# mahyarnajibi/SNIPER

Measured on AMD Instinct MI355X. Metric: train chips/sec (512x512, R101), higher is better.
Workload: dtype f16; 1 GPU; ResNet-101 Faster-RCNN SNIPER 3-scale, batch 20 x 512x512 fp16 per GPU (BASELINE configs[1]); step = GPU anchor labelling + fwd + bwd + grad all-reduce + SGD on HBM-resident chips (epoch chip generation / box assignment and image decode+resize are outside the step); f16 MFMA operands, f32 accumulation / losses / master weights; chips_per_gpu=20, global_batch=20, parallelism=dp1

## Files before the change

sniper_amd/csrc/common.h:

```cpp
#pragma once
#include <hip/hip_runtime.h>
#include <stdint.h>
#include <stdio.h>
#include <stdlib.h>

#include "../../include/sniper_hip.h"

#define SN_EXPORT extern "C" __attribute__((visibility("default")))

void sn_set_error(const char *fmt, ...);

#define SN_REQUIRE(cond, ...)      \
  do {                             \
    if (!(cond)) {                 \
      sn_set_error(__VA_ARGS__);   \
      return SN_ERR_ARG;           \
    }                              \
  } while (0)

#define SN_CHECK_LAUNCH()                                                      \
  do {                                                                         \
    hipError_t e__ = hipGetLastError();                                        \
    if (e__ != hipSuccess) {                                                   \
      sn_set_error("%s:%d HIP launch failed: %s", __FILE__, __LINE__, hipGetErrorString(e__)); \
      return SN_ERR_HIP;                                                       \
    }                                                                          \
  } while (0)

#define SN_HIP(call)                                                           \
  do {                                                                         \
    hipError_t e__ = (call);                                                   \
    if (e__ != hipSuccess) {                                                   \
      sn_set_error("%s:%d %s: %s", __FILE__, __LINE__, #call, hipGetErrorString(e__)); \
      return SN_ERR_HIP;                                                       \
    }                                                                          \
  } while (0)

hipError_t sn_once_per_device_max_lds(const void *kernel, int bytes);
enum SnDebugOption { SN_OPT_PROPOSAL_FULL_SORT = 0, SN_OPT_NMS_FULL_MASK = 1, SN_OPT_CONV_NO_PERSIST = 2, SN_OPT_SOFTMAX_STRIDED = 3, SN_OPT_COUNT };
int sn_debug_get(SnDebugOption which);

static inline hipStream_t sn_stream(sn_stream_t s) { return (hipStream_t)s; }
static inline int sn_div_up(int a, int b) { return (a + b - 1) / b; }
static inline size_t sn_align(size_t x, size_t a = 256) { return (x + a - 1) / a * a; }

static inline int sn_env_int(const char *name, int dflt) {
  const char *v = getenv(name);
  return v && *v ? atoi(v) : dflt;
}
static inline int sn_conv_out(int in, int k, int stride, int pad, int dil) { return (in + 2 * pad - dil * (k - 1) - 1) / stride + 1; }
static inline int sn_blocks(long total, int cap) {
  const long b = (total + 255) / 256;
  return (int)(b < 1 ? 1 : (b > cap ? cap : b));
}

constexpr int kWave = 64;

typedef _Float16 half_t;
typedef _Float16 half8 __attribute__((ext_vector_type(8)));
typedef _Float16 half4 __attribute__((ext_vector_type(4)));
typedef float floatx4 __attribute__((ext_vector_type(4)));

__device__ __forceinline__ unsigned sn_float_key(float f) {
  const unsigned u = __float_as_uint(f);
  return (u & 0x80000000u) ? ~u : (u | 0x80000000u);
}

int sn_partial_sum(const float *part, int nblk, long n, float *dst, hipStream_t s);

struct SnDiv { unsigned mul, sh, d; };
static inline SnDiv sn_div_make(unsigned d) {
  SnDiv f;
  unsigned s = 0;
  while ((1ull << s) < d) ++s;
  f.mul = (unsigned)((((unsigned long long)1 << 32) * (((unsigned long long)1 << s) - d)) / d + 1);
  f.sh = s;
  f.d = d;
  return f;
}
__device__ __forceinline__ unsigned sn_div(unsigned n, const SnDiv f) { return (__umulhi(n, f.mul) + n) >> f.sh; }
__device__ __forceinline__ unsigned sn_divmod(unsigned n, const SnDiv f, unsigned &rem) {
  const unsigned q = sn_div(n, f);
  rem = n - q * f.d;
  return q;
}
```

sniper_amd/csrc/common.hip:

```cpp
#include "common.h"

#include <stdarg.h>
#include <stdlib.h>
#include <string.h>

#include <atomic>
#include <mutex>
#include <string>
#include <utility>
#include <vector>

static thread_local char g_err[512] = "";

void sn_set_error(const char *fmt, ...) {
  va_list ap;
  va_start(ap, fmt);
  vsnprintf(g_err, sizeof(g_err), fmt, ap);
  va_end(ap);
}

SN_EXPORT const char *sn_last_error(void) { return g_err; }
SN_EXPORT int sn_version(void) { return 100; }

hipError_t sn_once_per_device_max_lds(const void *kernel, int bytes) {
  static std::mutex mu;
  static std::vector<std::pair<const void *, int>> done;
  int dev = 0;
  hipError_t e = hipGetDevice(&dev);
  if (e != hipSuccess) return e;
  std::lock_guard<std::mutex> lock(mu);
  for (const auto &d : done)
    if (d.first == kernel && d.second == dev) return hipSuccess;
  e = hipFuncSetAttribute(kernel, hipFuncAttributeMaxDynamicSharedMemorySize, bytes);
  if (e == hipSuccess) done.emplace_back(kernel, dev);
  return e;
}

static std::atomic<int> g_debug[SN_OPT_COUNT];
static const char *const kDebugNames[SN_OPT_COUNT] = {"proposal_full_sort", "nms_full_mask", "conv_no_persist", "softmax_strided"};
static const char *const kDebugEnv[SN_OPT_COUNT] = {"SNIPER_FULL_SORT", "SNIPER_NMS_FULL", "SNIPER_CONV_NO_PERSIST", "SNIPER_SOFTMAX_STRIDED"};
namespace {
struct DebugInit {
  DebugInit() {
    for (int i = 0; i < SN_OPT_COUNT; ++i) g_debug[i].store(getenv(kDebugEnv[i]) != nullptr ? 1 : 0, std::memory_order_relaxed);
  }
} g_debug_init;
}

int sn_debug_get(SnDebugOption which) { return g_debug[which].load(std::memory_order_relaxed); }

__global__ __launch_bounds__(256) void partial_sum_kernel(const float *__restrict__ part, int nblk, long n, float *__restrict__ dst) {
  const long e = (long)blockIdx.x * 256 + threadIdx.x;
  if (e >= n) return;
  float s = 0.f;
  int k = 0;
  for (; k + 8 <= nblk; k += 8) {
    float v[8];
#pragma unroll
    for (int u = 0; u < 8; ++u) v[u] = part[(size_t)(k + u) * n + e];
#pragma unroll
    for (int u = 0; u < 8; ++u) s += v[u];
  }
  for (; k < nblk; ++k) s += part[(size_t)k * n + e];
  dst[e] += s;
}

int sn_partial_sum(const float *part, int nblk, long n, float *dst, hipStream_t s) {
  hipLaunchKernelGGL(partial_sum_kernel, dim3((unsigned)((n + 255) / 256)), dim3(256), 0, s, part, nblk, n, dst);
  SN_CHECK_LAUNCH();
  return SN_OK;
}

SN_EXPORT int sn_debug_option(const char *name, int value) {
  SN_REQUIRE(name, "sn_debug_option: null name");
  for (int i = 0; i < SN_OPT_COUNT; ++i)
    if (strcmp(name, kDebugNames[i]) == 0) {
      g_debug[i].store(value, std::memory_order_relaxed);
      return SN_OK;
    }
  SN_REQUIRE(false, "sn_debug_option: unknown option '%s'", name);
}
```

sniper_amd/csrc/roi_deform.hip:

```cpp
#include "common.h"
#include "deform_sample.h"
#include <type_traits>

#include <stdlib.h>


struct RoiGeom {
  int b;
  float wstart, hstart, sub_w, sub_h, roi_w, roi_h;
};

__device__ __forceinline__ RoiGeom roi_geom(const float *__restrict__ rois, const float *__restrict__ trans, int r, int ph,
                                            int pw, int P, int S, float scale, float trans_std) {
#pragma clang fp contract(off)
  const float *q = rois + (size_t)r * 5;
  RoiGeom g;
  g.b = (int)q[0];
  const float sw = roundf(q[1]) * scale - 0.5f, sh = roundf(q[2]) * scale - 0.5f;
  const float ew = (roundf(q[3]) + 1.f) * scale - 0.5f, eh = (roundf(q[4]) + 1.f) * scale - 0.5f;
  g.roi_w = fmaxf(ew - sw, 0.1f);
  g.roi_h = fmaxf(eh - sh, 0.1f);
  const float bin_w = g.roi_w / (float)P, bin_h = g.roi_h / (float)P;
  g.sub_w = bin_w / (float)S;
  g.sub_h = bin_h / (float)S;
// ... 792 lines not shown
    const float wy = tent_sum(ay, y);
    if (wy == 0.f) continue;
    for (int x = ax.lo; x <= ax.hi; ++x) {
      const float wgt = wy * tent_sum(ax, x);
      if (wgt == 0.f) continue;
      sum += wgt * (float)img[((size_t)y * W + x) * C];
    }
  }
  return sum;
}

template <bool WAVE_PER_BIN>
__global__ __launch_bounds__(256) void psroi_ps_fwd_kernel(const half_t *__restrict__ data, const float *__restrict__ rois,
                                                           const float *__restrict__ trans, half_t *__restrict__ out, int R, int H,
                                                           int W, int C, int P, int S, int G, int D, float scale, float trans_std, int gm) {
  if constexpr (WAVE_PER_BIN) {
    const long total = (long)R * P * P;
    const long wv = ((long)blockIdx.x * blockDim.x + threadIdx.x) >> 6;
    if (wv >= total) return;
    const int lane = threadIdx.x & 63;
    const int pw = (int)(wv % P), ph = (int)((wv / P) % P), r = (int)(wv / ((long)P * P));
    const RoiGeom g = roi_geom(rois, trans, r, ph, pw, P, S, scale, trans_std);
    const AxisSamples ax = axis_samples(g.wstart, g.sub_w, S, W), ay = axis_samples(g.hstart, g.sub_h, S, H);
    const int count = ax.n * ay.n;
    const float inv = count ? 1.f / (float)count : 0.f;
    const int gh = ps_group(ph, G, P), gw = ps_group(pw, G, P);
    const half_t *img = data + (size_t)g.b * H * W * C;
    for (int d = lane; d < D; d += 64) {
      const float sum = count ? ps_bin_value(ax, ay, img + ps_channel(d, gh, gw, G, D, gm), W, C) : 0.f;
      out[(size_t)wv * D + d] = (half_t)(sum * inv);
    }
  } else {
    const long total = (long)R * P * P * D;
    for (long i = (long)blockIdx.x * blockDim.x + threadIdx.x; i < total; i += (long)gridDim.x * blockDim.x) {
      const int d = (int)(i % D);
      long t = i / D;
      const int pw = (int)(t % P); t /= P;
      const int ph = (int)(t % P);
      const int r = (int)(t / P);
      const RoiGeom g = roi_geom(rois, trans, r, ph, pw, P, S, scale, trans_std);
      const AxisSamples ax = axis_samples(g.wstart, g.sub_w, S, W), ay = axis_samples(g.hstart, g.sub_h, S, H);
      const int count = ax.n * ay.n;
      const int c = ps_channel(d, ps_group(ph, G, P), ps_group(pw, G, P), G, D, gm);
      const float sum = count ? ps_bin_value(ax, ay, data + (size_t)g.b * H * W * C + c, W, C) : 0.f;
      out[i] = (half_t)(count ? sum / (float)count : 0.f);
    }
  }
}

template <bool GM>
__global__ __launch_bounds__(256) void psroi_ps_bwd_data_kernel(const half_t *__restrict__ dout, const float *__restrict__ rois,
                                                                const float *__restrict__ trans, const int4 *__restrict__ win,
                                                                void *__restrict__ d_data, int out_f32, int R, int H, int W, int C,
                                                                int P, int S, int G, int D, float scale, float trans_std) {
  __shared__ __attribute__((aligned(16))) float ent[256 * kEntStride];
  __shared__ int roi_list[256];
  __shared__ int bins[256];
  __shared__ int wave_cnt[4], ent_cnt[4], nb_s;
  const int PP = P * P;
  const int tid = threadIdx.x, lane = tid & 63, wave = tid >> 6;
  const unsigned long long lt = (1ull << lane) - 1ull;
  int x0, y0;
  tile_origin(W, x0, y0);
  const int b = blockIdx.y;
  int c, d, mygrp, g_lo, g_hi;
  bool active_c;
  if constexpr (GM) {
    c = blockIdx.z * 256 + tid;
    active_c = c < C;
    mygrp = active_c ? c / D : -1;
    d = active_c ? c - mygrp * D : 0;
    g_lo = (blockIdx.z * 256) / D;
    g_hi = min(G * G - 1, (blockIdx.z * 256 + 255) / D);
  } else {
    const int chunks = (D + 255) >> 8;
    mygrp = g_lo = g_hi = blockIdx.z / chunks;
    d = (blockIdx.z % chunks) * 256 + tid;
    active_c = d < D;
    c = (d * G + mygrp / G) * G + mygrp % G;
  }
  if (tid == 0) {
    int n = 0;
    for (int bin = 0; bin < PP; ++bin) {
      const int grp = ps_group(bin / P, G, P) * G + ps_group(bin % P, G, P);
      if (grp >= g_lo && grp <= g_hi) bins[n++] = bin;
    }
    nb_s = n;
  }
  __syncthreads();
  const int nb = nb_s;
  float acc[16];
#pragma unroll
  for (int k = 0; k < 16; ++k) acc[k] = 0.f;
  if (nb > 0) {
    for (int base = 0; base < R; base += 256) {
      const int total = tile_scan_rois(win, base, R, b, x0, y0, roi_list, wave_cnt);
      const int nitems = total * nb;
      for (int it0 = 0; it0 < nitems; it0 += 256) {
        const int item = it0 + tid;
        bool act = false;
        float Wx[4] = {0.f, 0.f, 0.f, 0.f}, Wy[4] = {0.f, 0.f, 0.f, 0.f};
        float inv = 0.f;
        int idx = 0, grp = 0;
        if (item < nitems) {
          const int r = roi_list[item / nb], bin = bins[item % nb];
          const int ph = bin / P, pw = bin - ph * P;
          if constexpr (GM) grp = ps_group(ph, G, P) * G + ps_group(pw, G, P);
          act = bin_tile_weights(roi_geom(rois, trans, r, ph, pw, P, S, scale, trans_std), S, H, W, x0, y0, Wx, Wy, inv);
          idx = r * PP + bin;
        }
        const unsigned long long am = __ballot(act);
        if (lane == 0) ent_cnt[wave] = __popcll(am);
        __syncthreads();
        int eoff, n_e;
        wave_prefix4(ent_cnt, wave, eoff, n_e);
        if (act) {
          float *e = ent + (size_t)(eoff + __popcll(am & lt)) * kEntStride;
          e[0] = __int_as_float(idx);
          if constexpr (GM) e[1] = __int_as_float(grp);
          *reinterpret_cast<float4 *>(e + 4) = make_float4(Wx[0] * inv, Wx[1] * inv, Wx[2] * inv, Wx[3] * inv);
          *reinterpret_cast<float4 *>(e + 8) = make_float4(Wy[0], Wy[1], Wy[2], Wy[3]);
        }
        __syncthreads();
        if constexpr (GM) {
          for (int e = 0; e < n_e; ++e) {
            const float *q = ent + e * kEntStride;
            if (__float_as_int(q[1]) != mygrp) continue;
            tile_fma(q, (float)dout[(size_t)__float_as_int(q[0]) * D + d], acc);
          }
        } else {
          tile_accumulate<half_t>(ent, n_e, dout, (size_t)D, d, active_c, acc);
        }
        __syncthreads();
      }
    }
  }
  if (active_c) tile_store(acc, d_data, out_f32, b, y0, x0, H, W, C, c);
}

__global__ __launch_bounds__(256) void psroi_ps_bwd_trans_kernel(const half_t *__restrict__ dout, const half_t *__restrict__ data,
                                                                 const float *__restrict__ rois, const float *__restrict__ trans,
                                                                 float *__restrict__ d_trans, int R, int H, int W, int C, int P,
                                                                 int S, int G, int D, float scale, float trans_std, int gm) {
  const long total = (long)R * P * P;
  const long wv = ((long)blockIdx.x * blockDim.x + threadIdx.x) >> 6;
  if (wv >= total) return;
  const int lane = threadIdx.x & 63;
  const int pw = (int)(wv % P), ph = (int)((wv / P) % P), r = (int)(wv / ((long)P * P));
  const RoiGeom g = roi_geom(rois, trans, r, ph, pw, P, S, scale, trans_std);
  const int gh = ps_group(ph, G, P), gw = ps_group(pw, G, P);
  const half_t *img = data + (size_t)g.b * H * W * C;
  const AxisSamples ax = axis_samples(g.wstart, g.sub_w, S, W), ay = axis_samples(g.hstart, g.sub_h, S, H);
  const int count = ax.n * ay.n;
  const int nx = count ? ax.hi - ax.lo + 1 : 0, ny = count ? ay.hi - ay.lo + 1 : 0;
  float gtx = 0.f, gty = 0.f;
  if (count && nx <= kWinMax && ny <= kWinMax) {
    const int q = lane & 7;
    const bool is_y = (lane >> 3) & 1;
    const float wl = is_y ? (q < ny ? tent_sum(ay, ay.lo + q) : 0.f) : (q < nx ? tent_sum(ax, ax.lo + q) : 0.f);
    const float dl = is_y ? (q < ny ? tent_dsum(ay, ay.lo + q) : 0.f) : (q < nx ? tent_dsum(ax, ax.lo + q) : 0.f);
    for (int d = lane; d < D + 63 - ((D - 1) & 63); d += 64) {
      const bool on = d < D;
      const int c = ps_channel(on ? d : 0, gh, gw, G, D, gm);
      const float dv = on ? (float)dout[(size_t)wv * D + d] : 0.f;
      float sx = 0.f, sy = 0.f;
      for (int qy = 0; qy < ny; ++qy) {
        const float wy = __builtin_bit_cast(float, __builtin_amdgcn_readlane(__builtin_bit_cast(int, wl), 8 + qy));
        const float dwy = __builtin_bit_cast(float, __builtin_amdgcn_readlane(__builtin_bit_cast(int, dl), 8 + qy));
        if (wy == 0.f && dwy == 0.f) continue;
        const half_t *row = img + ((size_t)(ay.lo + qy) * W + ax.lo) * C + c;
        for (int qx = 0; qx < nx; ++qx) {
          const float kx = wy * __builtin_bit_cast(float, __builtin_amdgcn_readlane(__builtin_bit_cast(int, dl), qx));
          const float ky = dwy * __builtin_bit_cast(float, __builtin_amdgcn_readlane(__builtin_bit_cast(int, wl), qx));
          if (kx == 0.f && ky == 0.f) continue;
          const float u = on ? (float)row[(size_t)qx * C] : 0.f;
          sx += kx * u;
          sy += ky * u;
        }
      }
      gtx += sx * dv;
      gty += sy * dv;
    }
  } else if (count) {
    for (int ih = 0; ih < S; ++ih) {
      for (int iw = 0; iw < S; ++iw) {
        float w = sample_pos(g.wstart, iw, g.sub_w), h = sample_pos(g.hstart, ih, g.sub_h);
        if (w < -0.5f || w > (float)W - 0.5f || h < -0.5f || h > (float)H - 0.5f) continue;
        w = fminf(fmaxf(w, 0.f), (float)W - 1.f);
        h = fminf(fmaxf(h, 0.f), (float)H - 1.f);
        const int xa = (int)floorf(w), xb = (int)ceilf(w), ya = (int)floorf(h), yb = (int)ceilf(h);
        const float dx = w - (float)xa, dy = h - (float)ya;
        for (int d = lane; d < D; d += 64) {
          const int c = ps_channel(d, gh, gw, G, D, gm);
          const float dv = (float)dout[(size_t)wv * D + d];
          const float U00 = (float)img[((size_t)ya * W + xa) * C + c], U01 = (float)img[((size_t)ya * W + xb) * C + c];
          const float U10 = (float)img[((size_t)yb * W + xa) * C + c], U11 = (float)img[((size_t)yb * W + xb) * C + c];
          gtx += (U11 * dy + U01 * (1.f - dy) - U10 * dy - U00 * (1.f - dy)) * dv;
          gty += (U11 * dx + U10 * (1.f - dx) - U01 * dx - U00 * (1.f - dx)) * dv;
        }
      }
    }
  }
  const float k = count ? trans_std / (float)count : 0.f;
  gtx *= k * g.roi_w;
  gty *= k * g.roi_h;
  for (int off = 32; off > 0; off >>= 1) {
    gtx += __shfl_xor(gtx, off, 64);
    gty += __shfl_xor(gty, off, 64);
  }
  if (lane == 0) {
    d_trans[(((size_t)r * 2 + 0) * P + ph) * P + pw] = gtx;
    d_trans[(((size_t)r * 2 + 1) * P + ph) * P + pw] = gty;
  }
}

SN_EXPORT int sn_psroi_pool_fwd(const void *data, const float *rois, const float *trans, void *out, int R, int H, int W,
                                int output_dim, int group_size, int pooled, int sample_per_part, float spatial_scale,
                                float trans_std, int group_major, sn_stream_t stream) {
  SN_REQUIRE(data && rois && out && R > 0 && output_dim > 0 && group_size > 0 && pooled > 0 && sample_per_part > 0 &&
                 sample_per_part <= kMaxS, "sn_psroi_pool_fwd: bad arguments (sample_per_part <= %d)", kMaxS);
  const int C = output_dim * group_size * group_size;
  if (output_dim >= 32) {
    const long waves = (long)R * pooled * pooled;
    hipLaunchKernelGGL(psroi_ps_fwd_kernel<true>, dim3((unsigned)((waves * 64 + 255) / 256)), dim3(256), 0, sn_stream(stream),
                       (const half_t *)data, rois, trans, (half_t *)out, R, H, W, C, pooled, sample_per_part, group_size, output_dim,
                       spatial_scale, trans_std, group_major ? 1 : 0);
  } else {
    hipLaunchKernelGGL(psroi_ps_fwd_kernel<false>, dim3(blocks_for((long)R * pooled * pooled * output_dim)), dim3(256), 0,
                       sn_stream(stream), (const half_t *)data, rois, trans, (half_t *)out, R, H, W, C, pooled, sample_per_part,
                       group_size, output_dim, spatial_scale, trans_std, group_major ? 1 : 0);
  }
  SN_CHECK_LAUNCH();
  return SN_OK;
}

SN_EXPORT int sn_psroi_pool_bwd(const void *dout, const void *data, const float *rois, const float *trans, void *d_data,
                                int d_data_f32, float *d_trans, int R, int B, int H, int W, int output_dim, int group_size,
                                int pooled, int sample_per_part, float spatial_scale, float trans_std, int group_major, void *ws,
                                sn_stream_t stream) {
  if (const int e = roi_bwd_check("sn_psroi_pool_bwd", output_dim > 0 && group_size > 0, dout, data, rois, trans, d_data, d_trans, ws, R,
                                  B, H, W, pooled, sample_per_part))
    return e;
  const int C = output_dim * group_size * group_size;
  const long gz = (long)group_size * group_size * sn_div_up(output_dim, 256);
  SN_REQUIRE(gz <= 65535 && B <= 65535, "sn_psroi_pool_bwd: grid too large");
  hipStream_t s = sn_stream(stream);
  int4 *win = (int4 *)ws;
  if (const int e = roi_bwd_windows(rois, trans, win, R, H, W, pooled, sample_per_part, spatial_scale, trans_std, s)) return e;
  const int tiles = sn_div_up(W, 4) * sn_div_up(H, 4);
  if (group_major)
    hipLaunchKernelGGL(psroi_ps_bwd_data_kernel<true>, dim3(tiles, B, (unsigned)sn_div_up(C, 256)), dim3(256), 0, s, (const half_t *)dout,
                       rois, trans, (const int4 *)win, d_data, d_data_f32, R, H, W, C, pooled, sample_per_part, group_size, output_dim,
                       spatial_scale, trans_std);
  else
    hipLaunchKernelGGL(psroi_ps_bwd_data_kernel<false>, dim3(tiles, B, (unsigned)gz), dim3(256), 0, s, (const half_t *)dout, rois, trans,
                       (const int4 *)win, d_data, d_data_f32, R, H, W, C, pooled, sample_per_part, group_size, output_dim,
                       spatial_scale, trans_std);
  SN_CHECK_LAUNCH();
  if (trans) {
    const long waves = (long)R * pooled * pooled;
    hipLaunchKernelGGL(psroi_ps_bwd_trans_kernel, dim3((unsigned)((waves * 64 + 255) / 256)), dim3(256), 0, s,
                       (const half_t *)dout, (const half_t *)data, rois, trans, d_trans, R, H, W, C, pooled, sample_per_part,
                       group_size, output_dim, spatial_scale, trans_std, group_major ? 1 : 0);
    SN_CHECK_LAUNCH();
  }
  return SN_OK;
}

template <typename TO>
__global__ __launch_bounds__(256) void deform_im2col_kernel(const half_t *__restrict__ data, const TO *__restrict__ offset,
                                                            half_t *__restrict__ col, int N, int H, int W, int C, int Ho, int Wo,
                                                            int KH, int KW, int stride, int pad, int dil, int DG, int off_ps,
                                                            SnDiv d_cpr, SnDiv d_T, SnDiv d_Wo, SnDiv d_Ho, SnDiv d_KW, SnDiv d_cg) {
  const int cpr = C >> 3, T = KH * KW;
  const long total = (long)N * Ho * Wo * T * cpr;
  for (long i = (long)blockIdx.x * blockDim.x + threadIdx.x; i < total; i += (long)gridDim.x * blockDim.x) {
    unsigned chq, tapu, oxu, oyu;
    const unsigned t = sn_divmod((unsigned)i, d_cpr, chq);
    const unsigned m = sn_divmod(t, d_T, tapu);
    const unsigned t2 = sn_divmod(m, d_Wo, oxu);
    const int n = (int)sn_divmod(t2, d_Ho, oyu);
    const int ch = (int)chq * 8, tap = (int)tapu, ox = (int)oxu, oy = (int)oyu;
    const int g = (int)sn_div((unsigned)ch, d_cg), kh = (int)sn_div((unsigned)tap, d_KW), kw = tap - kh * KW;
    const TO *op = offset + (size_t)m * off_ps + g * 2 * T + 2 * tap;
    const float py = (float)(oy * stride - pad + kh * dil) + (float)op[0], px = (float)(ox * stride - pad + kw * dil) + (float)op[1];
    const DeformSample s = deform_sample(py, px, H, W);
    half8 o = {0, 0, 0, 0, 0, 0, 0, 0};
    if (s.ok) {
      const half_t *img = data + (size_t)n * H * W * C + ch;
      const half8 v1 = *reinterpret_cast<const half8 *>(img + ((size_t)s.y0 * W + s.x0) * C);
      const half8 v2 = *reinterpret_cast<const half8 *>(img + ((size_t)s.y0 * W + s.x1) * C);
      const half8 v3 = *reinterpret_cast<const half8 *>(img + ((size_t)s.y1 * W + s.x0) * C);
      const half8 v4 = *reinterpret_cast<const half8 *>(img + ((size_t)s.y1 * W + s.x1) * C);
      const float w1 = (1.f - s.ly) * (1.f - s.lx), w2 = (1.f - s.ly) * s.lx, w3 = s.ly * (1.f - s.lx), w4 = s.ly * s.lx;
#pragma unroll
      for (int j = 0; j < 8; ++j)
        o[j] = (half_t)(w1 * (float)v1[j] + w2 * (float)v2[j] + w3 * (float)v3[j] + w4 * (float)v4[j]);
    }
    *reinterpret_cast<half8 *>(col + i * 8) = o;
  }
}

template <typename TO>
__global__ __launch_bounds__(256) void deform_col2im_offset_kernel(const half_t *__restrict__ dcol, const half_t *__restrict__ data,
                                                                   const TO *__restrict__ offset, TO *__restrict__ d_offset, int N,
                                                                   int H, int W, int C, int Ho, int Wo, int KH, int KW, int stride,
                                                                   int pad, int dil, int DG, int off_ps, SnDiv d_cpr, SnDiv d_T,
                                                                   SnDiv d_Wo, SnDiv d_Ho, SnDiv d_KW, SnDiv d_cg) {
  const int cpr = C >> 3, T = KH * KW, cg = C / DG, lpg = cg >> 3;
  const long total = (long)N * Ho * Wo * T * cpr;
  const long i = (long)blockIdx.x * blockDim.x + threadIdx.x;
  const bool active = i < total;
  const long ii = active ? i : total - 1;
  unsigned chq, tapu, oxu, oyu;
  const unsigned t = sn_divmod((unsigned)ii, d_cpr, chq);
  const unsigned m = sn_divmod(t, d_T, tapu);
  const unsigned t2 = sn_divmod(m, d_Wo, oxu);
  const int n = (int)sn_divmod(t2, d_Ho, oyu);
  const int ch = (int)chq * 8, tap = (int)tapu, ox = (int)oxu, oy = (int)oyu;
  const int g = (int)sn_div((unsigned)ch, d_cg), kh = (int)sn_div((unsigned)tap, d_KW), kw = tap - kh * KW;
  const TO *op = offset + (size_t)m * off_ps + g * 2 * T + 2 * tap;
  const float py = (float)(oy * stride - pad + kh * dil) + (float)op[0], px = (float)(ox * stride - pad + kw * dil) + (float)op[1];
  const DeformSample s = deform_sample(py, px, H, W);
  float gy = 0.f, gx = 0.f;
  if (active && s.ok) {
    const half8 go = *reinterpret_cast<const half8 *>(dcol + ii * 8);
    const size_t base = (size_t)n * H * W * C + ch;
    const half8 v1 = *reinterpret_cast<const half8 *>(data + base + ((size_t)s.y0 * W + s.x0) * C);
    const half8 v2 = *reinterpret_cast<const half8 *>(data + base + ((size_t)s.y0 * W + s.x1) * C);
    const half8 v3 = *reinterpret_cast<const half8 *>(data + base + ((size_t)s.y1 * W + s.x0) * C);
    const half8 v4 = *reinterpret_cast<const half8 *>(data + base + ((size_t)s.y1 * W + s.x1) * C);
#pragma unroll
    for (int j = 0; j < 8; ++j) {
      const float d = (float)go[j];
      const float a = (float)v1[j], b = (float)v2[j], c = (float)v3[j], e = (float)v4[j];
      gy += d * ((1.f - s.lx) * (c - a) + s.lx * (e - b));
      gx += d * ((1.f - s.ly) * (b - a) + s.ly * (e - c));
    }
  }
  for (int off = lpg >> 1; off > 0; off >>= 1) {
    gy += __shfl_xor(gy, off, 64);
    gx += __shfl_xor(gx, off, 64);
  }
  if (active && ((ch >> 3) & (lpg - 1)) == 0) {
    TO *dp = d_offset + (size_t)m * off_ps + g * 2 * T + 2 * tap;
    dp[0] = (TO)gy;
    dp[1] = (TO)gx;
  }
}

template <typename TO>
__global__ __launch_bounds__(256) void deform_col2im_data_mfma_kernel(const half_t *__restrict__ dcol, const TO *__restrict__ offset,
                                                                      void *__restrict__ d_data, int out_f32, int H, int W, int C,
                                                                      int Ho, int Wo, int KH, int KW, int stride, int pad, int dil,
                                                                      int DG, int off_ps, int slabs,
                                                                      const unsigned *__restrict__ dmax_bits) {
  __shared__ __attribute__((aligned(16))) half_t w_hi[16][kListPitch];
  __shared__ __attribute__((aligned(16))) half_t w_lo[16][kListPitch];
  __shared__ __attribute__((aligned(16))) int e_row[kListCap];
  __shared__ int seg_n[4];
  const int tid = threadIdx.x, lane = tid & 63, wave = tid >> 6, nwave = blockDim.x >> 6, nthr = blockDim.x;
  const int fr = lane & 15, kg = lane >> 4;
  const unsigned long long lt = (1ull << lane) - 1ull;
  const int T = KH * KW, cg = C / DG;
  const int tiles_x = (W + 3) >> 2;
  const int x0 = (int)(blockIdx.x % tiles_x) * 4, y0 = (int)(blockIdx.x / tiles_x) * 4;
  const int n = blockIdx.y, g = blockIdx.z / slabs, slab = blockIdx.z - g * slabs;
  const int cl0 = slab * nthr + wave * 64;
  int oy_lo = 0, oy_hi = Ho - 1, ox_lo = 0, ox_hi = Wo - 1;
  if (dmax_bits) {
    const float D = __uint_as_float(*dmax_bits);
    if (D < 1.0e6f) {
      const int Di = (int)ceilf(D) + 1, span = (KH > KW ? KH : KW) - 1;
      auto fdiv = [](int a, int b) { return a >= 0 ? a / b : -((-a + b - 1) / b); };
      oy_lo = max(0, -fdiv(-(y0 - Di + pad - span * dil), stride));
      oy_hi = min(Ho - 1, fdiv(y0 + 3 + Di + pad, stride));
      ox_lo = max(0, -fdiv(-(x0 - Di + pad - span * dil), stride));
      ox_hi = min(Wo - 1, fdiv(x0 + 3 + Di + pad, stride));
    }
  }
  const int wh = max(oy_hi - oy_lo + 1, 0), ww = max(ox_hi - ox_lo + 1, 0);
  const int cand = wh * ww * T, cand_full = Ho * Wo * T;
  floatx4 acc[4];
#pragma unroll
  for (int j = 0; j < 4; ++j) acc[j] = floatx4{0.f, 0.f, 0.f, 0.f};
  int cnt = 0;
  auto flush = [&]() {
    const int kend = (cnt + 31) & ~31;
    for (int i = tid; i < (kend - cnt) * 16; i += nthr) {
      const int e = cnt + i / 16, m = i & 15;
      w_hi[m][e] = (half_t)0;
      w_lo[m][e] = (half_t)0;
      if (m == 0) e_row[e] = 0;
    }
    __syncthreads();
    for (int k0 = 0; k0 < cnt; k0 += 32) {
      const half8 a_hi = *reinterpret_cast<const half8 *>(&w_hi[fr][k0 + kg * 8]);
      const half8 a_lo = *reinterpret_cast<const half8 *>(&w_lo[fr][k0 + kg * 8]);
      const int4 r0 = *reinterpret_cast<const int4 *>(&e_row[k0 + kg * 8]);
      const int4 r1 = *reinterpret_cast<const int4 *>(&e_row[k0 + kg * 8 + 4]);
      const int rows[8] = {r0.x, r0.y, r0.z, r0.w, r1.x, r1.y, r1.z, r1.w};
      half8 bv[4];
#pragma unroll
      for (int j = 0; j < 4; ++j) {
        const int cl = cl0 + j * 16 + fr;
#pragma unroll
        for (int t = 0; t < 8; ++t) bv[j][t] = cl < cg ? dcol[(size_t)rows[t] * C + g * cg + cl] : (half_t)0;
      }
#pragma unroll
      for (int j = 0; j < 4; ++j) {
        acc[j] = __builtin_amdgcn_mfma_f32_16x16x32_f16(a_hi, bv[j], acc[j], 0, 0, 0);
        acc[j] = __builtin_amdgcn_mfma_f32_16x16x32_f16(a_lo, bv[j], acc[j], 0, 0, 0);
      }
    }
    __syncthreads();
    cnt = 0;
  };
  for (int base = 0; base < cand; base += nthr) {
    if (cnt > kListCap - nthr) flush();
    const int widx = base + tid;
    int idx = 0;
    bool hit = false;
    float Wx[4] = {0.f, 0.f, 0.f, 0.f}, Wy[4] = {0.f, 0.f, 0.f, 0.f};
    if (widx < cand) {
      const int wl = widx / T, tap = widx - wl * T;
      const int oy = oy_lo + wl / ww, ox = ox_lo + wl % ww;
      const int ml = oy * Wo + ox;
      idx = ml * T + tap;
      const int kh = tap / KW, kw = tap - kh * KW;
      const TO *op = offset + ((size_t)n * Ho * Wo + ml) * off_ps + g * 2 * T + 2 * tap;
      const float py = (float)(oy * stride - pad + kh * dil) + (float)op[0];
      const float px = (float)(ox * stride - pad + kw * dil) + (float)op[1];
      const DeformSample s = deform_sample(py, px, H, W);
      if (s.ok && s.x1 >= x0 && s.x0 <= x0 + 3 && s.y1 >= y0 && s.y0 <= y0 + 3) {
#pragma unroll
        for (int k = 0; k < 4; ++k) {
          Wx[k] = (s.x0 - x0 == k ? 1.f - s.lx : 0.f) + (s.x1 - x0 == k ? s.lx : 0.f);
          Wy[k] = (s.y0 - y0 == k ? 1.f - s.ly : 0.f) + (s.y1 - y0 == k ? s.ly : 0.f);
        }
        if (s.x0 == s.x1) {
#pragma unroll
          for (int k = 0; k < 4; ++k) Wx[k] = (s.x0 - x0 == k ? 1.f : 0.f);
        }
        if (s.y0 == s.y1) {
#pragma unroll
          for (int k = 0; k < 4; ++k) Wy[k] = (s.y0 - y0 == k ? 1.f : 0.f);
        }
        hit = true;
      }
    }
    const unsigned long long m = __ballot(hit);
    if (lane == 0) seg_n[wave] = __popcll(m);
    __syncthreads();
    int eoff = cnt, added = 0;
    for (int k = 0; k < nwave; ++k) {
      const int nn = seg_n[k];
      eoff += k < wave ? nn : 0;
      added += nn;
    }
    if (hit) {
      const int pos = eoff + __popcll(m & lt);
      e_row[pos] = n * cand_full + idx;
#pragma unroll
      for (int cy = 0; cy < 4; ++cy)
#pragma unroll
        for (int cx = 0; cx < 4; ++cx) {
          const float w = Wy[cy] * Wx[cx];
          const half_t hi = (half_t)w;
          w_hi[cy * 4 + cx][pos] = hi;
          w_lo[cy * 4 + cx][pos] = (half_t)(w - (float)hi);
        }
    }
    cnt += added;
    __syncthreads();
  }
  flush();
  const int y = y0 + kg;
#pragma unroll
  for (int j = 0; j < 4; ++j) {
    const int cl = cl0 + j * 16 + fr;
    if (cl >= cg || y >= H) continue;
#pragma unroll
    for (int r = 0; r < 4; ++r) {
      const int x = x0 + r;
      if (x >= W) continue;
      const size_t o = (((size_t)n * H + y) * W + x) * C + g * cg + cl;
      if (out_f32) ((float *)d_data)[o] = acc[j][r];
      else ((half_t *)d_data)[o] = (half_t)acc[j][r];
    }
  }
}

SN_EXPORT int sn_deform_im2col(const void *data, const void *offset, void *col, int N, int H, int W, int C, int KH, int KW,
                               int stride, int pad, int dil, int deformable_groups, int offset_pix_stride, int offset_dtype,
                               sn_stream_t stream) {
  SN_REQUIRE(data && offset && col && C % 8 == 0 && deformable_groups > 0 && (C / deformable_groups) % 8 == 0,
             "sn_deform_im2col: bad arguments");
  const int Ho = sn_conv_out(H, KH, stride, pad, dil), Wo = sn_conv_out(W, KW, stride, pad, dil);
  const long total = (long)N * Ho * Wo * KH * KW * (C / 8);
  SN_REQUIRE(total < 2147483647L, "sn_deform_im2col: too many column elements for 32-bit indexing");
  const SnDiv d_cpr = sn_div_make(C / 8), d_T = sn_div_make(KH * KW), d_Wo = sn_div_make(Wo), d_Ho = sn_div_make(Ho),
              d_KW = sn_div_make(KW), d_cg = sn_div_make(C / deformable_groups);
  if (offset_dtype == 0)
    hipLaunchKernelGGL((deform_im2col_kernel<half_t>), dim3(blocks_for(total)), dim3(256), 0, sn_stream(stream),
                       (const half_t *)data, (const half_t *)offset, (half_t *)col, N, H, W, C, Ho, Wo, KH, KW, stride, pad, dil,
                       deformable_groups, offset_pix_stride, d_cpr, d_T, d_Wo, d_Ho, d_KW, d_cg);
  else
    hipLaunchKernelGGL((deform_im2col_kernel<float>), dim3(blocks_for(total)), dim3(256), 0, sn_stream(stream),
                       (const half_t *)data, (const float *)offset, (half_t *)col, N, H, W, C, Ho, Wo, KH, KW, stride, pad, dil,
                       deformable_groups, offset_pix_stride, d_cpr, d_T, d_Wo, d_Ho, d_KW, d_cg);
  SN_CHECK_LAUNCH();
  return SN_OK;
}

template <typename TO>
__global__ __launch_bounds__(256) void deform_absmax_kernel(const TO *__restrict__ offset, long rows, int cols, int ld,
                                                            unsigned *__restrict__ out) {
  float m = 0.f;
  const long total = rows * cols;
  for (long i = (long)blockIdx.x * blockDim.x + threadIdx.x; i < total; i += (long)gridDim.x * blockDim.x) {
    const long r = i / cols;
    const float v = fabsf((float)offset[r * ld + (i - r * cols)]);
    m = (v > m || v != v) ? (v != v ? INFINITY : v) : m;
  }
  for (int off = 32; off > 0; off >>= 1) m = fmaxf(m, __shfl_xor(m, off, 64));
  __shared__ float wmax[4];
  if ((threadIdx.x & 63) == 0) wmax[threadIdx.x >> 6] = m;
  __syncthreads();
  if (threadIdx.x == 0) {
    const float b = fmaxf(fmaxf(wmax[0], wmax[1]), fmaxf(wmax[2], wmax[3]));
    const unsigned bits = __float_as_uint(b);
    if (bits > *reinterpret_cast<volatile unsigned *>(out)) atomicMax(out, bits);
  }
}

SN_EXPORT int sn_deform_col2im(const void *dcol, const void *data, const void *offset, void *d_data, int d_data_f32,
                               void *d_offset, int N, int H, int W, int C, int KH, int KW, int stride, int pad, int dil,
                               int deformable_groups, int offset_pix_stride, int offset_dtype, void *ws, sn_stream_t stream) {
  SN_REQUIRE(dcol && data && offset && C % 8 == 0 && deformable_groups > 0 && N > 0, "sn_deform_col2im: bad arguments");
  SN_REQUIRE(C % deformable_groups == 0, "sn_deform_col2im: C must be a multiple of the deformable groups");
  const int cg = C / deformable_groups, lpg = cg / 8;
  const int Ho = sn_conv_out(H, KH, stride, pad, dil), Wo = sn_conv_out(W, KW, stride, pad, dil);
  SN_REQUIRE((long)N * Ho * Wo * KH * KW < 2147483647L, "sn_deform_col2im: too many sampling points");
  hipStream_t s = sn_stream(stream);
  if (d_offset) {
    SN_REQUIRE(lpg >= 1 && lpg <= 64 && (lpg & (lpg - 1)) == 0 && cg % 8 == 0,
               "sn_deform_col2im: channels per deformable group / 8 must be a power of two <= 64");
    const long total = (long)N * Ho * Wo * KH * KW * (C / 8);
    SN_REQUIRE(total < 2147483647L - 256, "sn_deform_col2im: too many column elements for 32-bit indexing");
    const SnDiv d_cpr = sn_div_make(C / 8), d_T = sn_div_make(KH * KW), d_Wo = sn_div_make(Wo), d_Ho = sn_div_make(Ho),
                d_KW = sn_div_make(KW), d_cg = sn_div_make(cg);
    if (offset_dtype == 0)
      hipLaunchKernelGGL((deform_col2im_offset_kernel<half_t>), dim3((unsigned)((total + 255) / 256)), dim3(256), 0, s,
                         (const half_t *)dcol, (const half_t *)data, (const half_t *)offset, (half_t *)d_offset, N, H, W, C, Ho, Wo,
                         KH, KW, stride, pad, dil, deformable_groups, offset_pix_stride, d_cpr, d_T, d_Wo, d_Ho, d_KW, d_cg);
    else
      hipLaunchKernelGGL((deform_col2im_offset_kernel<float>), dim3((unsigned)((total + 255) / 256)), dim3(256), 0, s,
                         (const half_t *)dcol, (const half_t *)data, (const float *)offset, (float *)d_offset, N, H, W, C, Ho, Wo,
                         KH, KW, stride, pad, dil, deformable_groups, offset_pix_stride, d_cpr, d_T, d_Wo, d_Ho, d_KW, d_cg);
    SN_CHECK_LAUNCH();
  }
  if (d_data) {
    const int bt = cg >= 256 ? 256 : sn_div_up(cg, 64) * 64, slabs = sn_div_up(cg, bt);
    const dim3 grid(sn_div_up(W, 4) * sn_div_up(H, 4), N, deformable_groups * slabs);
    unsigned *dmax = (unsigned *)ws;
    if (dmax) {
      SN_HIP(hipMemsetAsync(dmax, 0, sizeof(unsigned), s));
      const long rows = (long)N * Ho * Wo;
      const int cols = 2 * KH * KW * deformable_groups;
      const long want = (rows * cols + 255) / 256;
      const unsigned blocks = (unsigned)(want > 256 ? 256 : (want < 1 ? 1 : want));
      if (offset_dtype == 0)
        hipLaunchKernelGGL((deform_absmax_kernel<half_t>), dim3(blocks), dim3(256), 0, s, (const half_t *)offset, rows, cols,
                           offset_pix_stride, dmax);
      else
        hipLaunchKernelGGL((deform_absmax_kernel<float>), dim3(blocks), dim3(256), 0, s, (const float *)offset, rows, cols,
                           offset_pix_stride, dmax);
      SN_CHECK_LAUNCH();
    }
    if (offset_dtype == 0)
      hipLaunchKernelGGL((deform_col2im_data_mfma_kernel<half_t>), grid, dim3(bt), 0, s, (const half_t *)dcol,
                         (const half_t *)offset, d_data, d_data_f32, H, W, C, Ho, Wo, KH, KW, stride, pad, dil, deformable_groups,
                         offset_pix_stride, slabs, (const unsigned *)dmax);
    else
      hipLaunchKernelGGL((deform_col2im_data_mfma_kernel<float>), grid, dim3(bt), 0, s, (const half_t *)dcol,
                         (const float *)offset, d_data, d_data_f32, H, W, C, Ho, Wo, KH, KW, stride, pad, dil, deformable_groups,
                         offset_pix_stride, slabs, (const unsigned *)dmax);
    SN_CHECK_LAUNCH();
  }
  return SN_OK;
}
```

Baseline: 1000 chips/s.

## Rewrite deformable col2im data-grad kernel with LDS-staged transposed MFMA and fused absmax

Adds a new deform col2im data-gradient kernel that stages gathered dcol rows into swizzled LDS per wave. It reads them back with ds_read_tr16 transposed loads for 16x16x32 MFMA, builds bilinear weights as separable y/x factors, and software-pipelines global loads. It also folds the offset abs-max reduction into the offset-gradient kernel, which removes a separate launch. The old kernel is kept behind a debug option. The cost is extra dynamic LDS and a waves-per-EU hint, with risk from the added complexity.

```diff
diff --git a/sniper_amd/csrc/common.h b/sniper_amd/csrc/common.h
--- a/sniper_amd/csrc/common.h
+++ b/sniper_amd/csrc/common.h
@@ -37,7 +37,8 @@
   } while (0)
 
 hipError_t sn_once_per_device_max_lds(const void *kernel, int bytes);
-enum SnDebugOption { SN_OPT_PROPOSAL_FULL_SORT = 0, SN_OPT_NMS_FULL_MASK = 1, SN_OPT_CONV_NO_PERSIST = 2, SN_OPT_SOFTMAX_STRIDED = 3, SN_OPT_COUNT };
+enum SnDebugOption { SN_OPT_PROPOSAL_FULL_SORT = 0, SN_OPT_NMS_FULL_MASK = 1, SN_OPT_CONV_NO_PERSIST = 2, SN_OPT_SOFTMAX_STRIDED = 3,
+                     SN_OPT_DEFORM_COL2IM_V1 = 4, SN_OPT_COUNT };
 int sn_debug_get(SnDebugOption which);
 
 static inline hipStream_t sn_stream(sn_stream_t s) { return (hipStream_t)s; }
diff --git a/sniper_amd/csrc/common.hip b/sniper_amd/csrc/common.hip
--- a/sniper_amd/csrc/common.hip
+++ b/sniper_amd/csrc/common.hip
@@ -37,12 +37,14 @@
 }
 
 static std::atomic<int> g_debug[SN_OPT_COUNT];
-static const char *const kDebugNames[SN_OPT_COUNT] = {"proposal_full_sort", "nms_full_mask", "conv_no_persist", "softmax_strided"};
-static const char *const kDebugEnv[SN_OPT_COUNT] = {"SNIPER_FULL_SORT", "SNIPER_NMS_FULL", "SNIPER_CONV_NO_PERSIST", "SNIPER_SOFTMAX_STRIDED"};
+static const char *const kDebugNames[SN_OPT_COUNT] = {"proposal_full_sort", "nms_full_mask", "conv_no_persist", "softmax_strided",
+                                                   "deform_col2im_v1"};
+static const char *const kDebugEnv[SN_OPT_COUNT] = {"SNIPER_FULL_SORT", "SNIPER_NMS_FULL", "SNIPER_CONV_NO_PERSIST", "SNIPER_SOFTMAX_STRIDED",
+                                                 nullptr};
 namespace {
 struct DebugInit {
   DebugInit() {
-    for (int i = 0; i < SN_OPT_COUNT; ++i) g_debug[i].store(getenv(kDebugEnv[i]) != nullptr ? 1 : 0, std::memory_order_relaxed);
+    for (int i = 0; i < SN_OPT_COUNT; ++i) g_debug[i].store(kDebugEnv[i] && getenv(kDebugEnv[i]) != nullptr ? 1 : 0, std::memory_order_relaxed);
   }
 } g_debug_init;
 }
diff --git a/sniper_amd/csrc/roi_deform.hip b/sniper_amd/csrc/roi_deform.hip
--- a/sniper_amd/csrc/roi_deform.hip
+++ b/sniper_amd/csrc/roi_deform.hip
@@ -1118,11 +1118,33 @@
 }
 
 template <typename TO>
+__device__ __forceinline__ void deform_absmax_block(const TO *__restrict__ offset, long rows, int cols, int ld,
+                                                    unsigned *__restrict__ out, int block, int nblocks) {
+  float m = 0.f;
+  const long total = rows * cols;
+  for (long i = (long)block * 256 + threadIdx.x; i < total; i += (long)nblocks * 256) {
+    const long r = i / cols;
+    const float v = fabsf((float)offset[r * ld + (i - r * cols)]);
+    m = (v > m || v != v) ? (v != v ? INFINITY : v) : m;
+  }
+  for (int off = 32; off > 0; off >>= 1) m = fmaxf(m, __shfl_xor(m, off, 64));
+  __shared__ float wmax[4];
+  if ((threadIdx.x & 63) == 0) wmax[threadIdx.x >> 6] = m;
+  __syncthreads();
+  if (threadIdx.x == 0) {
+    const float b = fmaxf(fmaxf(wmax[0], wmax[1]), fmaxf(wmax[2], wmax[3]));
+    const unsigned bits = __float_as_uint(b);
+    if (bits > *reinterpret_cast<volatile unsigned *>(out)) atomicMax(out, bits);
+  }
+}
+
+template <typename TO, bool AMAX>
 __global__ __launch_bounds__(256) void deform_col2im_offset_kernel(const half_t *__restrict__ dcol, const half_t *__restrict__ data,
                                                                    const TO *__restrict__ offset, TO *__restrict__ d_offset, int N,
                                                                    int H, int W, int C, int Ho, int Wo, int KH, int KW, int stride,
                                                                    int pad, int dil, int DG, int off_ps, SnDiv d_cpr, SnDiv d_T,
-                                                                   SnDiv d_Wo, SnDiv d_Ho, SnDiv d_KW, SnDiv d_cg) {
+                                                                   SnDiv d_Wo, SnDiv d_Ho, SnDiv d_KW, SnDiv d_cg,
+                                                                   unsigned *__restrict__ amax) {
   const int cpr = C >> 3, T = KH * KW, cg = C / DG, lpg = cg >> 3;
   const long total = (long)N * Ho * Wo * T * cpr;
   const long i = (long)blockIdx.x * blockDim.x + threadIdx.x;
@@ -1163,14 +1185,18 @@
     dp[0] = (TO)gy;
     dp[1] = (TO)gx;
   }
+  if (AMAX) {
+    const int nb = min((int)gridDim.x, 256);
+    if ((int)blockIdx.x < nb) deform_absmax_block(offset, (long)N * Ho * Wo, 2 * T * DG, off_ps, amax, (int)blockIdx.x, nb);
+  }
 }
 
 template <typename TO>
-__global__ __launch_bounds__(256) void deform_col2im_data_mfma_kernel(const half_t *__restrict__ dcol, const TO *__restrict__ offset,
-                                                                      void *__restrict__ d_data, int out_f32, int H, int W, int C,
-                                                                      int Ho, int Wo, int KH, int KW, int stride, int pad, int dil,
-                                                                      int DG, int off_ps, int slabs,
-                                                                      const unsigned *__restrict__ dmax_bits) {
+__global__ __launch_bounds__(256) void deform_col2im_data_v1_kernel(const half_t *__restrict__ dcol, const TO *__restrict__ offset,
+                                                                    void *__restrict__ d_data, int out_f32, int H, int W, int C,
+                                                                    int Ho, int Wo, int KH, int KW, int stride, int pad, int dil,
+                                                                    int DG, int off_ps, int slabs,
+                                                                    const unsigned *__restrict__ dmax_bits) {
   __shared__ __attribute__((aligned(16))) half_t w_hi[16][kListPitch];
   __shared__ __attribute__((aligned(16))) half_t w_lo[16][kListPitch];
   __shared__ __attribute__((aligned(16))) int e_row[kListCap];
@@ -1307,6 +1333,231 @@
   }
 }
 
+constexpr int kDcPre = 8;
+constexpr int kDcStageHalfs = 32 * 64;
+
+__device__ __forceinline__ void deform_tile_weights(const DeformSample &s, int x0, int y0, float (&Wy)[4], float (&Wx)[4]) {
+#pragma unroll
+  for (int k = 0; k < 4; ++k) {
+    Wx[k] = (s.x0 - x0 == k ? 1.f - s.lx : 0.f) + (s.x1 - x0 == k ? s.lx : 0.f);
+    Wy[k] = (s.y0 - y0 == k ? 1.f - s.ly : 0.f) + (s.y1 - y0 == k ? s.ly : 0.f);
+  }
+  if (s.x0 == s.x1) {
+#pragma unroll
+    for (int k = 0; k < 4; ++k) Wx[k] = (s.x0 - x0 == k ? 1.f : 0.f);
+  }
+  if (s.y0 == s.y1) {
+#pragma unroll
+    for (int k = 0; k < 4; ++k) Wy[k] = (s.y0 - y0 == k ? 1.f : 0.f);
+  }
+}
+
+__device__ __forceinline__ SnDiv deform_div_make(unsigned d) {
+  SnDiv f;
+  const unsigned s = d > 1 ? 32 - __clz((int)(d - 1)) : 0;
+  f.mul = (unsigned)((((unsigned long long)1 << 32) * (((unsigned long long)1 << s) - d)) / d + 1);
+  f.sh = s;
+  f.d = d;
+  return f;
+}
+
+template <typename TO>
+__global__ __launch_bounds__(256) __attribute__((amdgpu_waves_per_eu(4))) void deform_col2im_data_mfma_kernel(const half_t *__restrict__ dcol, const TO *__restrict__ offset,
+                                                                      void *__restrict__ d_data, int out_f32, int H, int W, int C,
+                                                                      int Ho, int Wo, int KH, int KW, int stride, int pad, int dil,
+                                                                      int DG, int off_ps, int slabs,
+                                                                      const unsigned *__restrict__ dmax_bits) {
+  __shared__ __attribute__((aligned(16))) float wy[4][kListCap];
+  __shared__ __attribute__((aligned(16))) float wx[4][kListCap];
+  __shared__ __attribute__((aligned(16))) int e_row[kListCap];
+  __shared__ int seg_n[2][kDcPre][4];
+  extern __shared__ __attribute__((aligned(16))) half_t dc_stage[];
+  const int tid = threadIdx.x, lane = tid & 63, wave = tid >> 6, nwave = blockDim.x >> 6, nthr = blockDim.x;
+  const int fr = lane & 15, kg = lane >> 4;
+  const unsigned long long lt = (1ull << lane) - 1ull;
+  const int T = KH * KW, cg = C / DG;
+  const int tiles_x = (W + 3) >> 2;
+  const int x0 = (int)(blockIdx.x % tiles_x) * 4, y0 = (int)(blockIdx.x / tiles_x) * 4;
+  const int n = blockIdx.y, g = blockIdx.z / slabs, slab = blockIdx.z - g * slabs;
+  const int cl0 = slab * nthr + wave * 64;
+  int oy_lo = 0, oy_hi = Ho - 1, ox_lo = 0, ox_hi = Wo - 1;
+  if (dmax_bits) {
+    const float D = __uint_as_float(*dmax_bits);
+    if (D < 1.0e6f) {
+      const int Di = (int)ceilf(D) + 1, span = (KH > KW ? KH : KW) - 1;
+      auto fdiv = [](int a, int b) { return a >= 0 ? a / b : -((-a + b - 1) / b); };
+      oy_lo = max(0, -fdiv(-(y0 - Di + pad - span * dil), stride));
+      oy_hi = min(Ho - 1, fdiv(y0 + 3 + Di + pad, stride));
+      ox_lo = max(0, -fdiv(-(x0 - Di + pad - span * dil), stride));
+      ox_hi = min(Wo - 1, fdiv(x0 + 3 + Di + pad, stride));
+    }
+  }
+  const int wh = max(oy_hi - oy_lo + 1, 0), ww = max(ox_hi - ox_lo + 1, 0);
+  const int cand = wh * ww * T, cand_full = Ho * Wo * T;
+  floatx4 acc[4];
+#pragma unroll
+  for (int j = 0; j < 4; ++j) acc[j] = floatx4{0.f, 0.f, 0.f, 0.f};
+  int cnt = 0;
+
+  half_t *const img = dc_stage + wave * kDcStageHalfs;
+  const int lr = lane >> 3, lu = lane & 7;
+  const bool ch_ok = cl0 + lu * 8 < cg;
+  const half_t *const dsrc = dcol + g * cg + (ch_ok ? cl0 + lu * 8 : 0);
+  int wr_off[4];
+#pragma unroll
+  for (int i = 0; i < 4; ++i) {
+    const int r = lr + 8 * i, f = ((r >> 1) & 1) | (((r >> 3) & 1) << 1);
+    wr_off[i] = r * 64 + ((((lu >> 1) ^ f) << 1) | (lu & 1)) * 8;
+  }
+  const int tr_row = kg * 8 + (fr >> 2), tr_f = ((tr_row >> 1) & 1) | (((tr_row >> 3) & 1) << 1);
+  const int cy = fr >> 2, cx = fr & 3;
+  auto issue = [&](int kc, int kend, half8(&v)[4]) {
+#pragma unroll
+    for (int i = 0; i < 4; ++i) {
+      const int e = kc + lr + 8 * i;
+      const int row = e < kend ? e_row[min(e, kListCap - 1)] : 0;
+      v[i] = *reinterpret_cast<const half8 *>(dsrc + (size_t)row * C);
+    }
+  };
+  auto consume = [&](int kc, const half8(&v)[4]) {
+    const half8 zero8 = {0, 0, 0, 0, 0, 0, 0, 0};
+    __builtin_amdgcn_fence(__ATOMIC_RELEASE, "wavefront");
+    __builtin_amdgcn_wave_barrier();
+#pragma unroll
+    for (int i = 0; i < 4; ++i) *reinterpret_cast<half8 *>(img + wr_off[i]) = ch_ok ? v[i] : zero8;
+    const floatx4 ya = *reinterpret_cast<const floatx4 *>(&wy[cy][kc + kg * 8]);
+    const floatx4 yb = *reinterpret_cast<const floatx4 *>(&wy[cy][kc + kg * 8 + 4]);
+    const floatx4 xa = *reinterpret_cast<const floatx4 *>(&wx[cx][kc + kg * 8]);
+    const floatx4 xb = *reinterpret_cast<const floatx4 *>(&wx[cx][kc + kg * 8 + 4]);
+    half8 a_hi, a_lo;
+#pragma unroll
+    for (int t = 0; t < 8; ++t) {
+      const float w = (t < 4 ? ya[t & 3] : yb[t & 3]) * (t < 4 ? xa[t & 3] : xb[t & 3]);
+      const half_t hi = (half_t)w;
+      a_hi[t] = hi;
+      a_lo[t] = (half_t)(w - (float)hi);
+    }
+    asm volatile("s_waitcnt lgkmcnt(0)" ::: "memory");
+    __builtin_amdgcn_fence(__ATOMIC_RELEASE, "wavefront");
+    __builtin_amdgcn_wave_barrier();
+    typedef short short4v_ __attribute__((ext_vector_type(4)));
+    typedef __attribute__((address_space(3))) short4v_ *lds_v4;
+    half8 bv[4];
+#pragma unroll
+    for (int j = 0; j < 4; ++j) {
+      const half_t *p = img + tr_row * 64 + ((j ^ tr_f) * 16) + cx * 4;
+      union { short4v_ s[2]; half8 hh; } u;
+      u.s[0] = __builtin_amdgcn_ds_read_tr16_b64_v4i16((lds_v4)p);
+      u.s[1] = __builtin_amdgcn_ds_read_tr16_b64_v4i16((lds_v4)(p + 4 * 64));
+      bv[j] = u.hh;
+    }
+#pragma unroll
+    for (int j = 0; j < 4; ++j) {
+      acc[j] = __builtin_amdgcn_mfma_f32_16x16x32_f16(a_hi, bv[j], acc[j], 0, 0, 0);
+      acc[j] = __builtin_amdgcn_mfma_f32_16x16x32_f16(a_lo, bv[j], acc[j], 0, 0, 0);
+    }
+  };
+  auto flush = [&]() {
+    const int kend = (cnt + 31) & ~31;
+    for (int i = tid; i < (kend - cnt) * 4; i += nthr) {
+      const int e = cnt + (i >> 2), k = i & 3;
+      wy[k][e] = 0.f;
+      wx[k][e] = 0.f;
+      if (k == 0) e_row[e] = 0;
+    }
+    __syncthreads();
+    if (cnt > 0) {
+      half8 va[4], vb[4];
+      issue(0, kend, va);
+      for (int kc = 0; kc < cnt; kc += 64) {
+        issue(kc + 32, kend, vb);
+        consume(kc, va);
+        issue(kc + 64, kend, va);
+        if (kc + 32 < cnt) consume(kc + 32, vb);
+      }
+    }
+    __syncthreads();
+    cnt = 0;
+  };
+
+  const SnDiv d_T = deform_div_make((unsigned)T), d_KW = deform_div_make((unsigned)KW), d_ww = deform_div_make((unsigned)max(ww, 1));
+  int par = 0;
+  for (int base0 = 0; base0 < cand; base0 += kDcPre * nthr, par ^= 1) {
+    float py[kDcPre], px[kDcPre];
+    int idx[kDcPre];
+#pragma unroll
+    for (int u = 0; u < kDcPre; ++u) {
+      const int widx = min(base0 + u * nthr + tid, cand - 1);
+      const int wl = (int)sn_div((unsigned)widx, d_T), tap = widx - wl * T;
+      const int wr = (int)sn_div((unsigned)wl, d_ww);
+      const int oy = oy_lo + wr, ox = ox_lo + (wl - wr * ww);
+      const int ml = oy * Wo + ox;
+      idx[u] = ml * T + tap;
+      const int kh = (int)sn_div((unsigned)tap, d_KW), kw = tap - kh * KW;
+      const TO *op = offset + ((size_t)n * Ho * Wo + ml) * off_ps + g * 2 * T + 2 * tap;
+      py[u] = (float)(oy * stride - pad + kh * dil) + (float)op[0];
+      px[u] = (float)(ox * stride - pad + kw * dil) + (float)op[1];
+    }
+    unsigned hits = 0;
+    unsigned long long m[kDcPre];
+#pragma unroll
+    for (int u = 0; u < kDcPre; ++u) {
+      const DeformSample s = deform_sample(py[u], px[u], H, W);
+      const bool hit = base0 + u * nthr + tid < cand && s.ok && s.x1 >= x0 && s.x0 <= x0 + 3 && s.y1 >= y0 && s.y0 <= y0 + 3;
+      hits |= hit ? 1u << u : 0u;
+      m[u] = __ballot(hit);
+      if (lane == 0) seg_n[par][u][wave] = __popcll(m[u]);
+    }
+    __syncthreads();
+#pragma unroll 1
+    for (int u = 0; u < kDcPre && base0 + u * nthr < cand; ++u) {
+      if (cnt > kListCap - nthr) flush();
+      int eoff = cnt, added = 0;
+      for (int k = 0; k < nwave; ++k) {
+        const int nn = seg_n[par][u][k];
+        eoff += k < wave ? nn : 0;
+        added += nn;
+      }
+      if (hits & 1u) {
+        const int pos = eoff + __popcll(m[0] & lt);
+        const DeformSample s = deform_sample(py[0], px[0], H, W);
+        float Wy[4], Wx[4];
+        deform_tile_weights(s, x0, y0, Wy, Wx);
+        e_row[pos] = n * cand_full + idx[0];
+#pragma unroll
+        for (int k = 0; k < 4; ++k) {
+          wy[k][pos] = Wy[k];
+          wx[k][pos] = Wx[k];
+        }
+      }
+      cnt += added;
+      hits >>= 1;
+#pragma unroll
+      for (int k = 0; k + 1 < kDcPre; ++k) {
+        py[k] = py[k + 1];
+        px[k] = px[k + 1];
+        idx[k] = idx[k + 1];
+        m[k] = m[k + 1];
+      }
+    }
+  }
+  flush();
+  const int y = y0 + kg;
+#pragma unroll
+  for (int j = 0; j < 4; ++j) {
+    const int cl = cl0 + j * 16 + fr;
+    if (cl >= cg || y >= H) continue;
+#pragma unroll
+    for (int r = 0; r < 4; ++r) {
+      const int x = x0 + r;
+      if (x >= W) continue;
+      const size_t o = (((size_t)n * H + y) * W + x) * C + g * cg + cl;
+      if (out_f32) ((float *)d_data)[o] = acc[j][r];
+      else ((half_t *)d_data)[o] = (half_t)acc[j][r];
+    }
+  }
+}
+
 SN_EXPORT int sn_deform_im2col(const void *data, const void *offset, void *col, int N, int H, int W, int C, int KH, int KW,
                                int stride, int pad, int dil, int deformable_groups, int offset_pix_stride, int offset_dtype,
                                sn_stream_t stream) {
@@ -1332,22 +1583,7 @@
 template <typename TO>
 __global__ __launch_bounds__(256) void deform_absmax_kernel(const TO *__restrict__ offset, long rows, int cols, int ld,
                                                             unsigned *__restrict__ out) {
-  float m = 0.f;
-  const long total = rows * cols;
-  for (long i = (long)blockIdx.x * blockDim.x + threadIdx.x; i < total; i += (long)gridDim.x * blockDim.x) {
-    const long r = i / cols;
-    const float v = fabsf((float)offset[r * ld + (i - r * cols)]);
-    m = (v > m || v != v) ? (v != v ? INFINITY : v) : m;
-  }
-  for (int off = 32; off > 0; off >>= 1) m = fmaxf(m, __shfl_xor(m, off, 64));
-  __shared__ float wmax[4];
-  if ((threadIdx.x & 63) == 0) wmax[threadIdx.x >> 6] = m;
-  __syncthreads();
-  if (threadIdx.x == 0) {
-    const float b = fmaxf(fmaxf(wmax[0], wmax[1]), fmaxf(wmax[2], wmax[3]));
-    const unsigned bits = __float_as_uint(b);
-    if (bits > *reinterpret_cast<volatile unsigned *>(out)) atomicMax(out, bits);
-  }
+  deform_absmax_block(offset, rows, cols, ld, out, (int)blockIdx.x, (int)gridDim.x);
 }
 
 SN_EXPORT int sn_deform_col2im(const void *dcol, const void *data, const void *offset, void *d_data, int d_data_f32,
@@ -1359,6 +1595,10 @@
   const int Ho = sn_conv_out(H, KH, stride, pad, dil), Wo = sn_conv_out(W, KW, stride, pad, dil);
   SN_REQUIRE((long)N * Ho * Wo * KH * KW < 2147483647L, "sn_deform_col2im: too many sampling points");
   hipStream_t s = sn_stream(stream);
+  const bool v1 = sn_debug_get(SN_OPT_DEFORM_COL2IM_V1) != 0;
+  unsigned *dmax = d_data ? (unsigned *)ws : nullptr;
+  const bool fused_max = dmax && d_offset && !v1;
+  if (dmax) SN_HIP(hipMemsetAsync(dmax, 0, sizeof(unsigned), s));
   if (d_offset) {
     SN_REQUIRE(lpg >= 1 && lpg <= 64 && (lpg & (lpg - 1)) == 0 && cg % 8 == 0,
                "sn_deform_col2im: channels per deformable group / 8 must be a power of two <= 64");
@@ -1366,22 +1606,25 @@
     SN_REQUIRE(total < 2147483647L - 256, "sn_deform_col2im: too many column elements for 32-bit indexing");
     const SnDiv d_cpr = sn_div_make(C / 8), d_T = sn_div_make(KH * KW), d_Wo = sn_div_make(Wo), d_Ho = sn_div_make(Ho),
                 d_KW = sn_div_make(KW), d_cg = sn_div_make(cg);
-    if (offset_dtype == 0)
-      hipLaunchKernelGGL((deform_col2im_offset_kernel<half_t>), dim3((unsigned)((total + 255) / 256)), dim3(256), 0, s,
-                         (const half_t *)dcol, (const half_t *)data, (const half_t *)offset, (half_t *)d_offset, N, H, W, C, Ho, Wo,
-                         KH, KW, stride, pad, dil, deformable_groups, offset_pix_stride, d_cpr, d_T, d_Wo, d_Ho, d_KW, d_cg);
-    else
-      hipLaunchKernelGGL((deform_col2im_offset_kernel<float>), dim3((unsigned)((total + 255) / 256)), dim3(256), 0, s,
-                         (const half_t *)dcol, (const half_t *)data, (const float *)offset, (float *)d_offset, N, H, W, C, Ho, Wo,
-                         KH, KW, stride, pad, dil, deformable_groups, offset_pix_stride, d_cpr, d_T, d_Wo, d_Ho, d_KW, d_cg);
+    const dim3 grid((unsigned)((total + 255) / 256));
+#define SN_DEFORM_OFFSET_LAUNCH(TO, AMAX)                                                                                          \
+  hipLaunchKernelGGL((deform_col2im_offset_kernel<TO, AMAX>), grid, dim3(256), 0, s, (const half_t *)dcol, (const half_t *)data, \
+                     (const TO *)offset, (TO *)d_offset, N, H, W, C, Ho, Wo, KH, KW, stride, pad, dil, deformable_groups,        \
+                     offset_pix_stride, d_cpr, d_T, d_Wo, d_Ho, d_KW, d_cg, dmax)
+    if (offset_dtype == 0) {
+      if (fused_max) SN_DEFORM_OFFSET_LAUNCH(half_t, true);
+      else SN_DEFORM_OFFSET_LAUNCH(half_t, false);
+    } else {
+      if (fused_max) SN_DEFORM_OFFSET_LAUNCH(float, true);
+      else SN_DEFORM_OFFSET_LAUNCH(float, false);
+    }
+#undef SN_DEFORM_OFFSET_LAUNCH
     SN_CHECK_LAUNCH();
   }
   if (d_data) {
     const int bt = cg >= 256 ? 256 : sn_div_up(cg, 64) * 64, slabs = sn_div_up(cg, bt);
     const dim3 grid(sn_div_up(W, 4) * sn_div_up(H, 4), N, deformable_groups * slabs);
-    unsigned *dmax = (unsigned *)ws;
-    if (dmax) {
-      SN_HIP(hipMemsetAsync(dmax, 0, sizeof(unsigned), s));
+    if (dmax && !fused_max) {
       const long rows = (long)N * Ho * Wo;
       const int cols = 2 * KH * KW * deformable_groups;
       const long want = (rows * cols + 255) / 256;
@@ -1394,14 +1637,18 @@
                            offset_pix_stride, dmax);
       SN_CHECK_LAUNCH();
     }
-    if (offset_dtype == 0)
-      hipLaunchKernelGGL((deform_col2im_data_mfma_kernel<half_t>), grid, dim3(bt), 0, s, (const half_t *)dcol,
-                         (const half_t *)offset, d_data, d_data_f32, H, W, C, Ho, Wo, KH, KW, stride, pad, dil, deformable_groups,
-                         offset_pix_stride, slabs, (const unsigned *)dmax);
-    else
-      hipLaunchKernelGGL((deform_col2im_data_mfma_kernel<float>), grid, dim3(bt), 0, s, (const half_t *)dcol,
-                         (const float *)offset, d_data, d_data_f32, H, W, C, Ho, Wo, KH, KW, stride, pad, dil, deformable_groups,
-                         offset_pix_stride, slabs, (const unsigned *)dmax);
+#define SN_DEFORM_DATA_LAUNCH(KERNEL, TO, LDS)                                                                                  \
+  hipLaunchKernelGGL((KERNEL<TO>), grid, dim3(bt), LDS, s, (const half_t *)dcol, (const TO *)offset, d_data, d_data_f32, H, W, \
+                     C, Ho, Wo, KH, KW, stride, pad, dil, deformable_groups, offset_pix_stride, slabs, (const unsigned *)dmax)
+    const size_t stage = (size_t)(bt / 64) * kDcStageHalfs * sizeof(half_t);
+    if (v1 || cg % 8 != 0) {
+      if (offset_dtype == 0) SN_DEFORM_DATA_LAUNCH(deform_col2im_data_v1_kernel, half_t, 0);
+      else SN_DEFORM_DATA_LAUNCH(deform_col2im_data_v1_kernel, float, 0);
+    } else {
+      if (offset_dtype == 0) SN_DEFORM_DATA_LAUNCH(deform_col2im_data_mfma_kernel, half_t, stage);
+      else SN_DEFORM_DATA_LAUNCH(deform_col2im_data_mfma_kernel, float, stage);
+    }
+#undef SN_DEFORM_DATA_LAUNCH
     SN_CHECK_LAUNCH();
   }
   return SN_OK;
```

Measured after the change: 1009 chips/s (median of 6 runs). No clear change (+0.9%).
